# Ascend-Research/HeadPoseEstimation-WHENet

Hardware: NVIDIA H100
Metric: head-crops/sec @224x224 bf16 (higher is better)
Workload: dtype bf16

## Files before the change

### headposeestimation-whenet_b200/build.py

```python
from __future__ import annotations

import os
import subprocess
import sys

HERE = os.path.dirname(os.path.abspath(__file__))
CSRC = os.path.join(HERE, "csrc")
OBJ = os.path.join(CSRC, "obj")
LIB = os.path.join(HERE, "libwhenet_b200.so")
_SIMT_TC = ["kernels_simt.cuh", "kernels_tc.cuh"]
_ABI = os.path.join("..", "..", "include", "whenet_b200.h")
UNITS = {
    "whenet_api.cu": _SIMT_TC + ["api_error.h", "kernels_fused.cuh", "kernels_crop.cuh", "kernels_k2.cuh", "kernels_tc32.cuh", "kernels_dwse.cuh", _ABI],
    "inst_k1_bf16.cu": _SIMT_TC + ["kernels_fused.cuh"],
    "inst_k1_f16.cu": _SIMT_TC + ["kernels_fused.cuh"],
    "inst_dwse.cu": _SIMT_TC + ["kernels_fused.cuh", "kernels_dwse.cuh"],
    "inst_pw.cu": _SIMT_TC + ["kernels_fused.cuh", "kernels_k2.cuh"],
    "inst_yolo.cu": _SIMT_TC + ["kernels_yolo.cuh"],
    "yolo_api.cu": _SIMT_TC + ["kernels_yolo.cuh", "api_error.h", _ABI],
}
SOURCES = list(UNITS)
HEADERS = sorted({h for hs in UNITS.values() for h in hs})

NVCC_FLAGS = ["-O3", "-std=c++17", "-gencode", "arch=compute_90a,code=sm_90a", "-lineinfo", "-Xcompiler", "-fPIC"]


def _obj(src: str) -> str:
    return os.path.join(OBJ, os.path.splitext(src)[0] + ".o")


def _unit_stale(src: str) -> bool:
    o = _obj(src)
    if not os.path.exists(o):
        return True
    t = os.path.getmtime(o)
    deps = [os.path.join(CSRC, d) for d in [src] + UNITS[src]] + [os.path.abspath(__file__)]
    return any(os.path.exists(d) and os.path.getmtime(d) > t for d in deps)


def _stale() -> bool:
    if not os.path.exists(LIB):
        return True
    t = os.path.getmtime(LIB)
    deps = [os.path.join(CSRC, d) for d in SOURCES + HEADERS] + [os.path.abspath(__file__)]
    return any(os.path.exists(d) and os.path.getmtime(d) > t for d in deps)


# ... 31 lines not shown
```

### headposeestimation-whenet_b200/csrc/inst_k1_bf16.cu

```cuda
#include "kernels_fused.cuh"

namespace whenet {
namespace fused {
template int launch_k1<__nv_bfloat16>(cudaStream_t, K1Params, int, int, int, int, size_t, int);
template int launch_dw_only<__nv_bfloat16>(cudaStream_t, K1Params, size_t, int);
}
}
```

### headposeestimation-whenet_b200/csrc/kernels_fused.cuh

```cuda
#pragma once
#include <algorithm>

#include "kernels_tc.cuh"

namespace whenet {
namespace fused {

using tc::BK;
using tc::BM;

constexpr size_t K1_MAX_SMEM = 227 * 1024 - 256;
constexpr float kDwScale = 4.0f;

struct K1Params {
    const void* in;
    const void* wt_aug;
    const float* w_dw;
    const void* w_dw16;
    const float* b_dw;
    void* out;
    float* partial;
    const float *w_se1t, *b_se1, *w_se2, *b_se2;
    float* gate;
    int* se_counter;
// ... 38 lines not shown
}
__device__ __forceinline__ void ffma2(float2& d, const float2& a, const float2& b) {
    d.x = fmaf(a.x, b.x, d.x);
    d.y = fmaf(a.y, b.y, d.y);
}
template <typename T> __device__ __forceinline__ void unpack2(uint32_t u, float& lo, float& hi);
template <> __device__ __forceinline__ void unpack2<__nv_bfloat16>(uint32_t u, float& lo, float& hi) {
    lo = __uint_as_float(u << 16);
    hi = __uint_as_float(u & 0xffff0000u);
}
template <> __device__ __forceinline__ void unpack2<__half>(uint32_t u, float& lo, float& hi) {
    const float2 f = __half22float2(*reinterpret_cast<const __half2*>(&u));
    lo = f.x; hi = f.y;
}
template <typename T> __device__ __forceinline__ uint32_t pack2(float lo, float hi);
template <> __device__ __forceinline__ uint32_t pack2<__nv_bfloat16>(float lo, float hi) {
    const __nv_bfloat162 h = __floats2bfloat162_rn(lo, hi);
    return *reinterpret_cast<const uint32_t*>(&h);
}
template <> __device__ __forceinline__ uint32_t pack2<__half>(float lo, float hi) {
    const __half2 h = __floats2half2_rn(lo, hi);
    return *reinterpret_cast<const uint32_t*>(&h);
}
template <typename T> __device__ __forceinline__ uint32_t ones2();
template <> __device__ __forceinline__ uint32_t ones2<__nv_bfloat16>() { return 0x3f803f80u; }
template <> __device__ __forceinline__ uint32_t ones2<__half>() { return 0x3c003c00u; }

__device__ __forceinline__ uint32_t sw128(int r, int c) {
    return (uint32_t)((r >> 3) * 1024 + (r & 7) * 128 + ((c ^ (r & 7)) << 4));
}

__device__ __forceinline__ int div_small(int x, float inv) { return __float2int_rz(((float)x + 0.5f) * inv); }

template <typename T, int KS, int S, int R, bool NOEXP = false, int CCT = 0, int NT = 256>
__global__ void __launch_bounds__(NT, NT == 256 ? 2 : 1) k1_expand_dw_kernel(const K1Params p) {
    const int CC = CCT ? CCT : p.CC;
    const int pitchE = CCT ? CCT * 2 + 16 : p.pitchE;
    constexpr bool HDW = !NOEXP && std::is_same<T, __nv_bfloat16>::value;
    constexpr int NG = NT / 128;
    extern __shared__ uint8_t smem_raw[];
    __shared__ int s_last;

    const int tid = threadIdx.x, warp = tid >> 5, lane = tid & 31;
    const uint32_t smem0 = (tc::smem_u32(smem_raw) + 1023u) & ~1023u;
    const uint32_t sA = smem0;
    const uint32_t sW = sA + p.smem_A;
    const uint32_t sC = sW + 2 * p.smem_W;
    const uint32_t sE = sC + 2 * p.smem_C;
    const uint32_t sR = sE + p.smem_E;
    float* const sM = reinterpret_cast<float*>(smem_raw + (sR + (uint32_t)(p.PY * CC) * 4u - tc::smem_u32(smem_raw)));

    const T* in = reinterpret_cast<const T*>(p.in);
    const T* wt = reinterpret_cast<const T*>(p.wt_aug);
    T* out = reinterpret_cast<T*>(p.out);

    const int n0 = blockIdx.y * p.NB, tile = blockIdx.x;
    const int nb_here = min(p.NB, p.N - n0);
    const int tyi = div_small(tile, 1.0f / (float)p.tiles_x);
    const int ty0 = tyi * p.TH, tx0 = (tile - tyi * p.tiles_x) * p.TW;
    const int iy0 = ty0 * S - p.pad, ix0 = tx0 * S - p.pad;
    const int npix = p.IH * p.IW;
    const int ty_lo = max(0, -iy0), tx_lo = max(0, -ix0);
    const int IHin = min(p.IH, p.Hin - iy0) - ty_lo, IWin = min(p.IW, p.Hin - ix0) - tx_lo;
    const int npix_in = IHin * IWin;
    const int rows_gemm = nb_here * npix_in;
    const float inv_IWin = 1.0f / (float)IWin, inv_npix = 1.0f / (float)npix_in;
// ... 92 lines not shown
    const int nstrips = p.TH << p.spr_log2;
    const uint32_t e_rowstride = (uint32_t)p.IW * pitchE;
    constexpr int NCOL = (R - 1) * S + KS;
    T* const out_n = out + (long long)(n0 + jc) * p.Ho * p.Ho * p.Cexp;

    asm volatile("cp.async.wait_group 0;" ::: "memory");
    asm volatile("fence.proxy.async.shared::cta;" ::: "memory");
    __syncthreads();
    constexpr bool BF16 = std::is_same<T, __nv_bfloat16>::value;
    const int nch16 = CC >> 4;
    constexpr int kMaxPieces = CCT ? CCT / 16 : 8;

    for (int ch = ch_begin; ch < ch_end; ++ch) {
        const int buf = ch & 1;
        const int cbase = ch * CC;
        if (!NOEXP) {
            for (int u = grp; u * 64 < rows_gemm; u += NG) {
                float d[8 * kMaxPieces];
                if constexpr (CCT != 0) {
                    tc::wg_mma_m64<BF16, CCT>(d, sA + (uint32_t)u * 64 * 128, a_kb_stride, sW + buf * p.smem_W, (uint32_t)CC * 128, p.cpr >> 1);
                } else {
#pragma unroll
                    for (int jj = 0; jj < kMaxPieces; ++jj)
                        if (jj < nch16)
                            tc::wg_mma_m64<BF16, 16>(*reinterpret_cast<float(*)[8]>(d + 8 * jj), sA + (uint32_t)u * 64 * 128, a_kb_stride,
                                                     sW + buf * p.smem_W + (uint32_t)jj * 2048u, (uint32_t)CC * 128, p.cpr >> 1);
                }
                tc::wg_wait<0>();
                const int r_lo = u * 64 + 16 * wq + (lane >> 2), cq = 2 * (lane & 3);
#pragma unroll
                for (int hr = 0; hr < 2; ++hr) {
                    const int r = r_lo + 8 * hr;
                    if (r < rows_gemm) {
                        const uint32_t er = e_row_of(r);
#pragma unroll
                        for (int jj = 0; jj < kMaxPieces; ++jj) {
                            if (jj < nch16) {
#pragma unroll
                                for (int i = 0; i < 2; ++i) {
                                    const uint32_t v = pack2<__half>(swish_from_half(d[8 * jj + 4 * i + 2 * hr]), swish_from_half(d[8 * jj + 4 * i + 2 * hr + 1]));
                                    asm volatile("st.shared.b32 [%0], %1;" ::"r"(er + (uint32_t)(16 * jj + 8 * i + cq) * 2u), "r"(v) : "memory");
                                }
                            }
                        }
                    }
                }
            }
        }
        if (ch + 1 < ch_end) prefetch_c(ch + 1, buf ^ 1);
        asm volatile("cp.async.commit_group;" ::: "memory");
        asm volatile("cp.async.wait_group 0;" ::: "memory");
        asm volatile("fence.proxy.async.shared::cta;" ::: "memory");
        __syncthreads();
        if (ch + 2 < ch_end) prefetch_w(ch + 2, buf);
        asm volatile("cp.async.commit_group;" ::: "memory");

        float sum[4] = {0.f, 0.f, 0.f, 0.f};
        if (dw_active) {
            const int c0 = cbase + cv * 4;
            const uint32_t cst = sC + buf * p.smem_C + (uint32_t)cv * 16;
            const float4 bq = lds_f4(cst);
            const uint32_t e_cv = sE + (uint32_t)(jc * p.e_rows) * pitchE + (uint32_t)cv * 8;
            for (int sidx = pl; sidx < nstrips; sidx += p.PYc) {
                const int oyl = sidx >> p.spr_log2, oxl0 = (sidx - (oyl << p.spr_log2)) * R;
                float2 acc[R][2];
                uint32_t erow = e_cv + (uint32_t)(oyl * S) * e_rowstride + (uint32_t)(oxl0 * S) * pitchE;
                using TE = typename std::conditional<NOEXP, T, __half>::type;
                if constexpr (!HDW) {
#pragma unroll
                    for (int r = 0; r < R; ++r) { acc[r][0] = make_float2(bq.x, bq.y); acc[r][1] = make_float2(bq.z, bq.w); }
#pragma unroll
                    for (int ky = 0; ky < KS; ++ky) {
                        float2 wr[KS][2];
#pragma unroll
                        for (int kx = 0; kx < KS; ++kx) {
                            const float4 wq = lds_f4(cst + (uint32_t)((1 + ky * KS + kx) * CC) * 4);
                            wr[kx][0] = make_float2(wq.x, wq.y); wr[kx][1] = make_float2(wq.z, wq.w);
                        }
                        uint32_t ea = erow;
#pragma unroll
                        for (int col = 0; col < NCOL; ++col) {
                            uint32_t a, b;
                            lds64(ea, a, b);
                            ea += pitchE;
                            float2 x01, x23;
                            unpack2<TE>(a, x01.x, x01.y);
                            unpack2<TE>(b, x23.x, x23.y);
#pragma unroll
                            for (int r = 0; r < R; ++r) {
                                const int kx = col - r * S;
                                if (kx >= 0 && kx < KS) {
                                    ffma2(acc[r][0], x01, wr[kx][0]);
                                    ffma2(acc[r][1], x23, wr[kx][1]);
                                }
                            }
                        }
                        erow += e_rowstride;
                    }
                } else {
                    __half2 hacc[R][2];
#pragma unroll
                    for (int r = 0; r < R; ++r) { hacc[r][0] = __float2half2_rn(0.f); hacc[r][1] = __float2half2_rn(0.f); }
                    const uint32_t cst_h = cst - (uint32_t)cv * 16 + (uint32_t)CC * 4 + (uint32_t)cv * 8;
#pragma unroll
                    for (int ky = 0; ky < KS; ++ky) {
                        __half2 wr[KS][2];
#pragma unroll
                        for (int kx = 0; kx < KS; ++kx) {
                            uint32_t w0, w1;
                            lds64(cst_h + (uint32_t)((ky * KS + kx) * CC) * 2, w0, w1);
                            wr[kx][0] = *reinterpret_cast<__half2*>(&w0); wr[kx][1] = *reinterpret_cast<__half2*>(&w1);
                        }
                        uint32_t ea = erow;
#pragma unroll
                        for (int col = 0; col < NCOL; ++col) {
                            uint32_t a, b;
                            lds64(ea, a, b);
                            ea += pitchE;
                            const __half2 x01 = *reinterpret_cast<__half2*>(&a), x23 = *reinterpret_cast<__half2*>(&b);
#pragma unroll
                            for (int r = 0; r < R; ++r) {
                                const int kx = col - r * S;
                                if (kx >= 0 && kx < KS) {
                                    hacc[r][0] = __hfma2(x01, wr[kx][0], hacc[r][0]);
                                    hacc[r][1] = __hfma2(x23, wr[kx][1], hacc[r][1]);
                                }
                            }
                        }
                        erow += e_rowstride;
                    }
                    const float2 sc = make_float2(kDwScale, kDwScale);
#pragma unroll
                    for (int r = 0; r < R; ++r) {
                        acc[r][0] = make_float2(bq.x, bq.y); acc[r][1] = make_float2(bq.z, bq.w);
                        ffma2(acc[r][0], __half22float2(hacc[r][0]), sc);
                        ffma2(acc[r][1], __half22float2(hacc[r][1]), sc);
                    }
                }
                const int oy = ty0 + oyl;
                T* dst = out_n + ((long long)oy * p.Ho + tx0 + oxl0) * p.Cexp + c0;
#pragma unroll
                for (int r = 0; r < R; ++r) {
                    if (oxl0 + r < p.TW && oy < p.Ho && tx0 + oxl0 + r < p.Ho) {
#pragma unroll
                        for (int i = 0; i < 2; ++i) {
                            acc[r][i].x = swish_from_half(acc[r][i].x); acc[r][i].y = swish_from_half(acc[r][i].y);
                            sum[2 * i] += acc[r][i].x; sum[2 * i + 1] += acc[r][i].y;
                        }
                        uint2 o;
                        o.x = pack2<T>(acc[r][0].x, acc[r][0].y);
                        o.y = pack2<T>(acc[r][1].x, acc[r][1].y);
                        *reinterpret_cast<uint2*>(dst + (long long)r * p.Cexp) = o;
                    }
                }
            }
            asm volatile("st.shared.v4.f32 [%0], {%1,%2,%3,%4};" ::"r"(sR + (uint32_t)(py * CC + cv * 4) * 4),
                         "f"(sum[0]), "f"(sum[1]), "f"(sum[2]), "f"(sum[3]) : "memory");
        }
        __syncthreads();
        if (tid < p.NB * CC) {
            const int jj = tid >= CC ? 1 : 0, cc = tid - jj * CC;
            if (jj < nb_here) {
                float s4[4] = {0.f, 0.f, 0.f, 0.f};
                const uint32_t r0 = sR + (uint32_t)(jj * p.PYc * CC + cc) * 4;
                int y = 0;
                for (; y + 3 < p.PYc; y += 4) {
#pragma unroll
                    for (int i = 0; i < 4; ++i) {
                        float t;
                        asm volatile("ld.shared.f32 %0, [%1];" : "=f"(t) : "r"(r0 + (uint32_t)((y + i) * CC) * 4));
                        s4[i] += t;
                    }
                }
                for (; y < p.PYc; ++y) {
                    float t;
                    asm volatile("ld.shared.f32 %0, [%1];" : "=f"(t) : "r"(r0 + (uint32_t)(y * CC) * 4));
                    s4[y & 3] += t;
                }
                const float tot = (s4[0] + s4[1]) + (s4[2] + s4[3]);
                p.partial[((long long)(n0 + jj) * gridDim.x + tile) * p.Cexp + cbase + cc] = tot;
                if (p.se_tail) sM[jj * p.Cexp + cbase + cc] = tot * p.inv_hw;
            }
        }
        __syncthreads();
    }
    if (p.se_counter) __threadfence();
    __syncthreads();
// ... 202 lines not shown
```

### headposeestimation-whenet_b200/csrc/whenet_api.cu

```cuda
#include <cuda_bf16.h>
#include <cuda_fp16.h>
#include <cuda_runtime.h>

#include <algorithm>
#include <atomic>
#include <cmath>
#include <cstdarg>
#include <cstdio>
#include <cstdlib>
#include <cstring>
#include <map>
#include <string>
#include <thread>
#include <type_traits>
#include <vector>

#include "../../include/whenet_b200.h"
#include "api_error.h"
#include "kernels_simt.cuh"
#include "kernels_tc.cuh"
#include "kernels_fused.cuh"
#include "kernels_crop.cuh"
#include "kernels_k2.cuh"
#include "kernels_tc32.cuh"
#include "kernels_dwse.cuh"
#include <cudaTypedefs.h>

namespace whenet {
namespace fused {
#define WHENET_EXTERN_FUSED(T)                                                                            \
    extern template int launch_k1<T>(cudaStream_t, K1Params, int, int, int, int, size_t, int);            \
    extern template int launch_dw_only<T>(cudaStream_t, K1Params, size_t, int);
WHENET_EXTERN_FUSED(__nv_bfloat16)
WHENET_EXTERN_FUSED(__half)
#undef WHENET_EXTERN_FUSED
extern template int launch_dwse<__nv_bfloat16>(cudaStream_t, DwSeParams, int, int, int, int, int);
extern template int launch_dwse_x<__nv_bfloat16>(cudaStream_t, DwSeParams, int, int, int, int, int);
extern template int launch_dwse_spatial<__nv_bfloat16>(cudaStream_t, DwSeParams, int, int, int);
}
namespace tc {
#define WHENET_EXTERN_PW(T)                                                                                                         \
    extern template int launch_pw_tc2<T>(cudaStream_t, const T*, const void*, const float*, const float*, const T*, T*, long long, \
                                         int, int, int, bool, int, int, int, bool);                                                 \
    extern template int launch_k2<T>(cudaStream_t, const K2Params&, size_t, bool, bool, bool, int);          \
    extern template int launch_pw_tc3<T>(cudaStream_t, const T*, const void*, const float*, const float*, const T*, T*, long long, int, int, int);
WHENET_EXTERN_PW(__nv_bfloat16)
WHENET_EXTERN_PW(__half)
#undef WHENET_EXTERN_PW
}
}

namespace {

using whenet::api::fail;
using whenet::api::g_err;

#define CK(call)                                                                                   \
    do {                                                                                           \
        cudaError_t e__ = (call);                                                                  \
        if (e__ != cudaSuccess)                                                                    \
            return fail(WHENET_ECUDA, "%s failed at %s:%d: %s", #call, __FILE__, __LINE__,         \
                        cudaGetErrorString(e__));                                                  \
    } while (0)

constexpr double kBnEps = 1e-3;
constexpr int kImgElems = 224 * 224 * 3;

struct BlockCfg {
    int idx, hin, hout, cin, cexp, cout, k, s, cse, pad;
    bool skip, has_expand;
};
// ... 51 lines not shown
struct GraphEntry { GraphKey key; cudaGraphExec_t exec; int launches; };
struct EvPair { cudaEvent_t a, b; int stat; };
struct Stat { std::string name; double bytes = 0, flops = 0; int launches = 0; float ms = 0; };

}

struct whenet_ctx {
    int device = 0, max_batch = 0, precision = 0;
    int chunk = 0;
    int use_tc = 0;
    int* h_tflag = nullptr;
    int* d_tflag = nullptr;
    int dw_variant = 1;
    int pw_variant = 4;
    std::map<TmapKey, CUtensorMap> tmaps2;
    int pw_stage_cap = 0, pw_smem_kb = 54, pw_min_ctas = 132;
    int stem_variant = 1;
    whenet::StemParams stem_params{};
    bool async_host = false;
    unsigned host_pass_ctr = 0;
    float* d_angles_slot[2] = {nullptr, nullptr};
    float* d_logits_slot[2] = {nullptr, nullptr};
    int host_chunk = 1 << 30;
    int cfg_epoch = 0;
    int use_graph = 0;
    std::vector<GraphEntry> graphs;
    int use_fused = 0;
    int fused_max_block = 16;
    int kd_tail = 0;
    int se_batch = 1;
    int pw3 = 1;
    int dw1_kd = 1;
    int head_batch = 1;
    int kd_from = 7;
    std::vector<K1Plan> k1;
    std::map<TmapKey, CUtensorMap> tmaps;
    int sm_count = 132;
    K1Plan dw1;
    int dw1_fused = 1;
    cudaStream_t own_stream = nullptr, stream = nullptr, copy_stream = nullptr;
    bool weights_loaded = false;
    std::vector<BlockCfg> blocks;
    std::vector<BlockW> bw;
    float* d_arena = nullptr;
    void* d_arena16 = nullptr;
    size_t split_lo_bytes = 0;
    std::vector<int64_t> layout;
    float *w_stem = nullptr, *b_stem = nullptr, *lut = nullptr;
    float *w_head = nullptr, *b_head = nullptr, *w_fct = nullptr, *b_fc = nullptr;
    void* wt_head = nullptr;
    int ws_chunk = 0;
    size_t ws_io = 0, ws_ex = 0, ws_dw = 0, ws_part = 0;
    cudaStream_t aux_stream[4] = {nullptr, nullptr, nullptr, nullptr};
    cudaEvent_t ev_fork = nullptr, ev_join[4] = {nullptr, nullptr, nullptr, nullptr}, ev_half[4] = {nullptr, nullptr, nullptr, nullptr};
    int n_streams = 2;
    void *bufA = nullptr, *bufB = nullptr, *bufE = nullptr, *bufD = nullptr;
    float *d_partial = nullptr, *d_gate = nullptr, *d_angles = nullptr, *d_logits = nullptr, *d_pooled = nullptr;
    int* d_se_counter = nullptr;
    int se_wide = 0;
    int se_scale_out = 1;
    int k1_split_ctas = 120;
    int se_tail = 1;
    int se_fused = 0;
    void* d_in[2] = {nullptr, nullptr};
    void* h_stage = nullptr;
    size_t h_stage_bytes = 0;
// ... 141 lines not shown
    static PFN_cuTensorMapEncodeTiled_v12000 fn = nullptr;
    if (!fn) {
        void* f = nullptr;
        cudaDriverEntryPointQueryResult q;
        if (cudaGetDriverEntryPoint("cuTensorMapEncodeTiled", &f, cudaEnableDefault, &q) == cudaSuccess && q == cudaDriverEntryPointSuccess)
            fn = reinterpret_cast<PFN_cuTensorMapEncodeTiled_v12000>(f);
    }
    return fn;
}
int make_tmap_w(CUtensorMap* tm, const void* base, int rows, int K, int box_rows, bool is_bf16) {
    auto fn = tmap_encode_fn();
    if (!fn) return fail(WHENET_ECUDA, "cuTensorMapEncodeTiled is not available from this driver");
    const cuuint64_t dims[2] = {(cuuint64_t)K, (cuuint64_t)rows};
    const cuuint64_t strides[1] = {(cuuint64_t)K * 2};
    const cuuint32_t box[2] = {64, (cuuint32_t)box_rows};
    const cuuint32_t estr[2] = {1, 1};
    const CUresult r = fn(tm, is_bf16 ? CU_TENSOR_MAP_DATA_TYPE_BFLOAT16 : CU_TENSOR_MAP_DATA_TYPE_FLOAT16, 2, const_cast<void*>(base), dims, strides,
                          box, estr, CU_TENSOR_MAP_INTERLEAVE_NONE, CU_TENSOR_MAP_SWIZZLE_128B, CU_TENSOR_MAP_L2_PROMOTION_L2_256B,
                          CU_TENSOR_MAP_FLOAT_OOB_FILL_NONE);
    if (r != CUDA_SUCCESS) return fail(WHENET_ECUDA, "cuTensorMapEncodeTiled(weights %dx%d, box %d) failed: %d", rows, K, box_rows, (int)r);
    return 0;
}

int make_tmap_kd_e(CUtensorMap* tm, const void* base, int n, int H, int C, int cc, int pw) {
    auto fn = tmap_encode_fn();
    if (!fn) return fail(WHENET_ECUDA, "cuTensorMapEncodeTiled is not available from this driver");
    const cuuint64_t dims[4] = {(cuuint64_t)C, (cuuint64_t)H, (cuuint64_t)H, (cuuint64_t)n};
    const cuuint64_t strides[3] = {(cuuint64_t)C * 2, (cuuint64_t)H * C * 2, (cuuint64_t)H * H * C * 2};
    const cuuint32_t box[4] = {(cuuint32_t)cc, (cuuint32_t)pw, (cuuint32_t)pw, 1};
    const cuuint32_t estr[4] = {1, 1, 1, 1};
    const CUresult r = fn(tm, CU_TENSOR_MAP_DATA_TYPE_FLOAT16, 4, const_cast<void*>(base), dims, strides, box, estr, CU_TENSOR_MAP_INTERLEAVE_NONE,
                          CU_TENSOR_MAP_SWIZZLE_NONE, CU_TENSOR_MAP_L2_PROMOTION_L2_128B, CU_TENSOR_MAP_FLOAT_OOB_FILL_NONE);
    if (r != CUDA_SUCCESS) return fail(WHENET_ECUDA, "cuTensorMapEncodeTiled(KD tile %dx%dx%dx%d, box %dx%dx%d) failed: %d", n, H, H, C, pw, pw, cc, (int)r);
    return 0;
}
int make_tmap_kd_w(CUtensorMap* tm, const void* base, int kk, int C, int cc) {
    auto fn = tmap_encode_fn();
    if (!fn) return fail(WHENET_ECUDA, "cuTensorMapEncodeTiled is not available from this driver");
    const cuuint64_t dims[2] = {(cuuint64_t)C, (cuuint64_t)kk};
    const cuuint64_t strides[1] = {(cuuint64_t)C * 2};
    const cuuint32_t box[2] = {(cuuint32_t)cc, (cuuint32_t)kk};
    const cuuint32_t estr[2] = {1, 1};
    const CUresult r = fn(tm, CU_TENSOR_MAP_DATA_TYPE_FLOAT16, 2, const_cast<void*>(base), dims, strides, box, estr, CU_TENSOR_MAP_INTERLEAVE_NONE,
                          CU_TENSOR_MAP_SWIZZLE_NONE, CU_TENSOR_MAP_L2_PROMOTION_L2_128B, CU_TENSOR_MAP_FLOAT_OOB_FILL_NONE);
    if (r != CUDA_SUCCESS) return fail(WHENET_ECUDA, "cuTensorMapEncodeTiled(KD weights %dx%d, box %d) failed: %d", kk, C, cc, (int)r);
    return 0;
}

template <typename T>
int launch_pw(whenet_ctx* c, const char* name, const T* A, const float* W, const void* Wt16, const float* bias,
              const float* gate, const T* resid, T* out, long long M, int K, int N, int hw, bool swish, bool out_half = false) {
    const double bytes = (double)M * (K + N + (resid ? N : 0)) * sizeof(T);
    const double flops = 2.0 * (double)M * K * N;
    Scope sc(c, name, bytes, flops);
    if constexpr (sizeof(T) == 2) {
        const bool want_k2 = c->pw_variant == 3 || (c->pw_variant == 4 && (gate == nullptr || hw <= 196));
        if (c->use_tc && Wt16 && want_k2 && !out_half) {
            whenet::tc::K2Params kp{};
            size_t smem = 0;
            if (whenet::tc::plan_k2(M, K, N, hw, gate != nullptr, c->precision == WHENET_PRECISION_BF16, &kp, &smem) &&
                (c->pw_variant == 3 || kp.tiles >= 2 * c->sm_count)) {
                if (c->tmaps2.size() > 1024) c->tmaps2.clear();
                const TmapKey ka{K, (int)M, (const void*)A}, kw{-N, K, Wt16};
                auto ia = c->tmaps2.find(ka);
                if (ia == c->tmaps2.end()) {
                    CUtensorMap tm;
// ... 235 lines not shown
                    if (rc != 0) return fail(WHENET_ECUDA, "KD (on-chip expand) launch failed for block %d (rc=%d)", b.idx, rc);
                    CK(cudaGetLastError());
                } else {
                    Scope sc(c, nm, (double)nb * ((double)b.hin * b.hin + (double)b.hout * b.hout) * b.cexp * sizeof(T),
                             2.0 * nb * (double)b.hout * b.hout * b.k * b.k * b.cexp);
                    rc = whenet::fused::launch_dwse<T>(c->stream, p, b.k, b.s, b.hin, nb, split);
                    if (rc != 0) return fail(WHENET_ECUDA, "KD launch failed for block %d (rc=%d)", b.idx, rc);
                    CK(cudaGetLastError());
                }
                tiles = 1;
                did_k1 = true;
              }
            } else if (c->use_fused && c->k1[i].valid && b.idx <= c->fused_max_block) {
                whenet::fused::K1Params p = c->k1[i].p;
                p.in = cur; p.wt_aug = w.wt_exp_aug; p.w_dw = w.w_dw_h; p.w_dw16 = w.w_dw16; p.b_dw = w.b_dw_h; p.out = D; p.partial = c->d_partial; p.tflag = c->d_tflag;
                p.w_se1t = w.w_se1t; p.b_se1 = w.b_se1; p.w_se2 = w.w_se2; p.b_se2 = w.b_se2; p.gate = c->d_gate; p.Cse = b.cse;
                se_in_k1 = c->se_fused && p.NB == 1;
                p.se_counter = se_in_k1 ? c->d_se_counter : nullptr;
                {
                    const long long ctas = (long long)p.tiles_x * p.tiles_y * ((nb + p.NB - 1) / p.NB);
                    int split = 1;
                    while (split < p.n_chunks && ctas * split < c->k1_split_ctas) ++split;
                    p.chunks_per_cta = (p.n_chunks + split - 1) / split;
                    if (c->se_tail && !se_in_k1 && p.tiles_x * p.tiles_y == 1 && split == 1) {
                        p.se_tail = 1;
                        p.inv_hw = 1.0f / (float)(b.hout * b.hout);
                        se_in_k1 = true;
                        if (c->se_scale_out && !taps) { p.scale_out = 1; d_gated = true; }
                    }
                }
                snprintf(nm, sizeof nm, "b%02d.k1", b.idx);
                Scope sc(c, nm, (double)nb * ((double)b.hin * b.hin * b.cin + (double)b.hout * b.hout * b.cexp) * sizeof(T),
                         2.0 * nb * ((double)b.hin * b.hin * b.cin * b.cexp + (double)b.hout * b.hout * b.k * b.k * b.cexp));
                int rc = whenet::fused::launch_k1<T>(c->stream, p, b.k, b.s, c->k1[i].R, c->k1[i].NT, c->k1[i].smem, nb);
                if (rc != 0) return fail(WHENET_ECUDA, "K1 launch failed for block %d (rc=%d)", b.idx, rc);
                CK(cudaGetLastError());
                tiles = p.tiles_x * p.tiles_y;
                did_k1 = true;
            }
        }
        if (!did_k1) {
        if (b.has_expand) {
            snprintf(nm, sizeof nm, "b%02d.expand", b.idx);
            int rc = launch_pw<T>(c, nm, cur, w.w_exp, w.wt_exp, w.b_exp, nullptr, nullptr, E,
                                  (long long)nb * b.hin * b.hin, b.cin, b.cexp, b.hin * b.hin, true);
            if (rc) return rc;
            dw_in = E;
        }
        snprintf(nm, sizeof nm, "b%02d.dw", b.idx);
        int rc = launch_dw<T>(c, nm, b, w, dw_in, D, nb, &tiles);
        if (rc) return rc;
        }
        int rc = 0;
        if (!se_in_k1) {
            snprintf(nm, sizeof nm, "b%02d.se", b.idx);
            Scope sc(c, nm, (double)nb * (tiles + 1) * b.cexp * 4.0, 4.0 * nb * b.cexp * b.cse);
            const float inv_hw = 1.0f / (float)(b.hout * b.hout);
            const size_t se_smem = (b.cexp + b.cse) * sizeof(float);
            if (nb >= 64 && c->se_batch) {
                constexpr int SEB = 4;
                whenet::se_gate_batch_kernel<SEB, 512><<<(nb + SEB - 1) / SEB, 512, SEB * se_smem, c->stream>>>(
                    c->d_partial, tiles, inv_hw, w.w_se1t, w.b_se1, w.w_se2, w.b_se2, c->d_gate, b.cexp, b.cse, nb);
            } else if (nb < 64 || c->se_wide)
                whenet::se_gate_kernel<1024><<<nb, 1024, se_smem, c->stream>>>(
                    c->d_partial, tiles, inv_hw, w.w_se1t, w.b_se1, w.w_se2, w.b_se2, c->d_gate, b.cexp, b.cse);
            else
                whenet::se_gate_kernel<256><<<nb, 256, se_smem, c->stream>>>(
                    c->d_partial, tiles, inv_hw, w.w_se1t, w.b_se1, w.w_se2, w.b_se2, c->d_gate, b.cexp, b.cse);
            CK(cudaGetLastError());
// ... 404 lines not shown
    if (prop.major != 9 || prop.minor != 0)
        return fail(WHENET_ECUDA, "device %d is sm_%d%d; this library is built for sm_90a (H100) only", device, prop.major, prop.minor);
    whenet_ctx* c = new whenet_ctx();
    c->device = device;
    c->max_batch = max_batch;
    c->precision = precision;
    c->sm_count = prop.multiProcessorCount;
    const char* ev = getenv("WHENET_CHUNK");
    int chunk = ev ? atoi(ev) : max_batch;
    if (chunk < 1) chunk = max_batch;
    c->chunk = std::min(chunk, max_batch);
    c->use_tc = precision != WHENET_PRECISION_FP32;
    if (const char* e2 = getenv("WHENET_TC")) c->use_tc = atoi(e2) && precision != WHENET_PRECISION_FP32;
    c->blocks = make_blocks();
    c->bw.resize(c->blocks.size());
    c->k1.resize(c->blocks.size());
    if (precision != WHENET_PRECISION_FP32) {
        const BlockCfg& b1 = c->blocks[0];
        c->dw1.valid = !b1.has_expand && whenet::fused::plan_dw_only(b1.hin, b1.cexp, b1.k, b1.s, b1.pad, &c->dw1.p, &c->dw1.smem);
        c->dw1.R = 7;
    }
    if (precision != WHENET_PRECISION_FP32)
        for (size_t i = 0; i < c->blocks.size(); ++i) {
            const BlockCfg& b = c->blocks[i];
            if (!b.has_expand) continue;
            K1Plan& pl = c->k1[i];
            whenet::fused::K1Choice ch{};
            pl.valid = whenet::fused::plan_k1(b.hin, b.hout, b.cin, b.cexp, b.k, b.s, b.pad, precision == WHENET_PRECISION_BF16, true,
                                              &pl.p, &ch, &pl.smem);
            pl.R = ch.r;
            pl.NT = ch.nt;
        }
    c->use_fused = precision != WHENET_PRECISION_FP32;
    if (const char* e3 = getenv("WHENET_FUSED")) c->use_fused = atoi(e3) && precision != WHENET_PRECISION_FP32;
    CK(cudaStreamCreateWithFlags(&c->own_stream, cudaStreamNonBlocking));
    CK(cudaStreamCreateWithFlags(&c->copy_stream, cudaStreamNonBlocking));
    c->stream = c->own_stream;
    CK(cudaEventCreateWithFlags(&c->ev_fork, cudaEventDisableTiming));
    for (int i = 0; i < 4; ++i) {
        CK(cudaStreamCreateWithFlags(&c->aux_stream[i], cudaStreamNonBlocking));
        CK(cudaEventCreateWithFlags(&c->ev_join[i], cudaEventDisableTiming));
        CK(cudaEventCreateWithFlags(&c->ev_half[i], cudaEventDisableTiming));
    }
    for (int i = 0; i < 2; ++i) {
        CK(cudaEventCreateWithFlags(&c->ev_ready[i], cudaEventDisableTiming));
        CK(cudaEventCreateWithFlags(&c->ev_free[i], cudaEventDisableTiming));
    }
    CK(cudaHostAlloc((void**)&c->h_tflag, sizeof(int), cudaHostAllocMapped));
    *c->h_tflag = 0;
    CK(cudaHostGetDevicePointer((void**)&c->d_tflag, c->h_tflag, 0));
    CK(cudaMalloc(&c->d_angles, (size_t)max_batch * 3 * sizeof(float) * 2));
    CK(cudaMalloc(&c->d_logits, (size_t)max_batch * WHENET_N_LOGITS * sizeof(float) * 2));
    for (int i = 0; i < 2; ++i) {
        c->d_angles_slot[i] = c->d_angles + (size_t)i * max_batch * 3;
        c->d_logits_slot[i] = c->d_logits + (size_t)i * max_batch * WHENET_N_LOGITS;
    }
    *out = c;
    return 0;
}

int whenet_load_weights(whenet_ctx* c, const whenet_tensor* tensors, int n_tensors) {
    if (!c || !tensors || n_tensors < 1) return fail(WHENET_EINVAL, "bad arguments");
    CK(cudaSetDevice(c->device));
    TensorMap tm;
    for (int i = 0; i < n_tensors; ++i)
        if (tensors[i].name) tm.m[tensors[i].name] = &tensors[i];
// ... 433 lines not shown
            out[n].ms = s.ms; out[n].launches = s.launches; out[n].bytes = s.bytes; out[n].flops = s.flops;
        }
        ++n;
    }
    if (out) { c->stats.clear(); c->stat_idx.clear(); }
    return n;
}

int64_t whenet_launch_count(whenet_ctx* c) { return c ? c->launches : 0; }

int whenet_set_option(whenet_ctx* c, const char* key, int value) {
    if (!c || !key) return fail(WHENET_EINVAL, "bad arguments");
    drop_graphs(c);
    c->cfg_epoch++;
    if (!strcmp(key, "tensor_cores")) { c->use_tc = value; return 0; }
    if (!strcmp(key, "streams")) { c->n_streams = value < 1 ? 1 : (value > 4 ? 4 : value); return 0; }
    if (!strcmp(key, "se_fused")) { c->se_fused = value; return 0; }
    if (!strcmp(key, "se_tail")) { c->se_tail = value; return 0; }
    if (!strcmp(key, "se_scale_out")) { c->se_scale_out = value; return 0; }
    if (!strcmp(key, "k1_split_ctas")) { c->k1_split_ctas = value; return 0; }
    if (!strcmp(key, "se_wide")) { c->se_wide = value; return 0; }
    if (!strcmp(key, "host_chunk")) { if (value < 1) return fail(WHENET_EINVAL, "host_chunk must be >= 1"); c->host_chunk = value; return 0; }
    if (!strcmp(key, "graph")) { c->use_graph = value; if (!value) drop_graphs(c); return 0; }
    if (!strcmp(key, "dw_variant")) { c->dw_variant = value; return 0; }
    if (!strcmp(key, "stem_variant")) { c->stem_variant = value; return 0; }
    if (!strcmp(key, "dw1_fused")) { c->dw1_fused = value; return 0; }
    if (!strcmp(key, "pw_variant")) { c->pw_variant = value; return 0; }
    if (!strcmp(key, "pw_stage_cap")) { c->pw_stage_cap = value; return 0; }
    if (!strcmp(key, "pw_smem_kb")) { c->pw_smem_kb = value; return 0; }
    if (!strcmp(key, "pw_min_ctas")) { c->pw_min_ctas = value; return 0; }
    if (!strcmp(key, "fused")) { c->use_fused = value && c->precision != WHENET_PRECISION_FP32; return 0; }
    if (!strcmp(key, "fused_max_block")) { c->fused_max_block = value; return 0; }
    if (!strcmp(key, "kd_from")) { c->kd_from = value; return 0; }
    if (!strcmp(key, "kd_tail")) { c->kd_tail = value; return 0; }
    if (!strcmp(key, "se_batch")) { c->se_batch = value; return 0; }
    if (!strcmp(key, "head_batch")) { c->head_batch = value; return 0; }
    if (!strcmp(key, "dw1_kd")) { c->dw1_kd = value; return 0; }
    if (!strcmp(key, "pw3")) { c->pw3 = value; return 0; }
    if (!strcmp(key, "stage_threads")) { c->stage_threads = value < 0 ? 0 : (value > 32 ? 32 : value); return 0; }
    if (!strcmp(key, "chunk")) {
        if (value < 1) return fail(WHENET_EINVAL, "chunk must be >= 1");
        c->chunk = std::min(value, c->max_batch);
        return 0;
    }
    return fail(WHENET_ENOTFOUND, "unknown option %s", key);
}

void whenet_destroy(whenet_ctx* c) {
    if (!c) return;
    cudaSetDevice(c->device);
    cudaDeviceSynchronize();
    drop_graphs(c);
    free_ws(c);
    if (c->d_frame) cudaFree(c->d_frame);
    if (c->d_rects) cudaFree(c->d_rects);
    if (c->d_frame_of) cudaFree(c->d_frame_of);
    for (auto& kv : c->taps) cudaFree(kv.second.first);
    for (auto& p : c->ev_used) { cudaEventDestroy(p.a); cudaEventDestroy(p.b); }
    for (auto e : c->ev_pool) cudaEventDestroy(e);
    if (c->d_arena) cudaFree(c->d_arena);
    if (c->d_arena16) cudaFree(c->d_arena16);
    if (c->d_angles) cudaFree(c->d_angles);
    if (c->d_logits) cudaFree(c->d_logits);
    if (c->h_tflag) cudaFreeHost(c->h_tflag);
    for (int i = 0; i < 2; ++i) {
        if (c->ev_ready[i]) cudaEventDestroy(c->ev_ready[i]);
// ... 17 lines not shown
```

Before: 74410.

## Add specialized TMA-fed expand+depthwise K1X kernel for bf16 blocks

Adds a new compile-time specialized kernel that fuses the expand GEMM (wgmma) and HFMA2 depthwise conv for selected block shapes. All operands are loaded by TMA with mbarrier pipelining: the input tile, double-buffered expand weights and double-buffered depthwise weights plus bias. It also factors the shared expand-store and depthwise strip code into helpers reused by the old kernel. The intent is to cut per-thread address math and manual staging loads and to overlap weight fetch with compute. The cost is more template instances, extra tensor-map management, and a path taken only when a shape instance matches.

```diff
diff --git a/headposeestimation-whenet_b200/build.py b/headposeestimation-whenet_b200/build.py
--- a/headposeestimation-whenet_b200/build.py
+++ b/headposeestimation-whenet_b200/build.py
@@ -11,8 +11,8 @@
 _SIMT_TC = ["kernels_simt.cuh", "kernels_tc.cuh"]
 _ABI = os.path.join("..", "..", "include", "whenet_b200.h")
 UNITS = {
-    "whenet_api.cu": _SIMT_TC + ["api_error.h", "kernels_fused.cuh", "kernels_crop.cuh", "kernels_k2.cuh", "kernels_tc32.cuh", "kernels_dwse.cuh", _ABI],
-    "inst_k1_bf16.cu": _SIMT_TC + ["kernels_fused.cuh"],
+    "whenet_api.cu": _SIMT_TC + ["api_error.h", "kernels_fused.cuh", "kernels_crop.cuh", "kernels_k2.cuh", "kernels_tc32.cuh", "kernels_dwse.cuh", "kernels_k1x.cuh", _ABI],
+    "inst_k1_bf16.cu": _SIMT_TC + ["kernels_fused.cuh", "kernels_dwse.cuh", "kernels_k1x.cuh"],
     "inst_k1_f16.cu": _SIMT_TC + ["kernels_fused.cuh"],
     "inst_dwse.cu": _SIMT_TC + ["kernels_fused.cuh", "kernels_dwse.cuh"],
     "inst_pw.cu": _SIMT_TC + ["kernels_fused.cuh", "kernels_k2.cuh"],
diff --git a/headposeestimation-whenet_b200/csrc/inst_k1_bf16.cu b/headposeestimation-whenet_b200/csrc/inst_k1_bf16.cu
--- a/headposeestimation-whenet_b200/csrc/inst_k1_bf16.cu
+++ b/headposeestimation-whenet_b200/csrc/inst_k1_bf16.cu
@@ -1,8 +1,10 @@
 #include "kernels_fused.cuh"
+#include "kernels_k1x.cuh"
 
 namespace whenet {
 namespace fused {
 template int launch_k1<__nv_bfloat16>(cudaStream_t, K1Params, int, int, int, int, size_t, int);
 template int launch_dw_only<__nv_bfloat16>(cudaStream_t, K1Params, size_t, int);
+template int launch_k1x<__nv_bfloat16>(cudaStream_t, DwSeParams, int, int, int, int, int, int, int, int);
 }
 }
diff --git a/headposeestimation-whenet_b200/csrc/kernels_fused.cuh b/headposeestimation-whenet_b200/csrc/kernels_fused.cuh
--- a/headposeestimation-whenet_b200/csrc/kernels_fused.cuh
+++ b/headposeestimation-whenet_b200/csrc/kernels_fused.cuh
@@ -94,6 +94,81 @@
 
 __device__ __forceinline__ int div_small(int x, float inv) { return __float2int_rz(((float)x + 0.5f) * inv); }
 
+template <int NP>
+__device__ __forceinline__ void expand_row_to_e(const float (&d)[8 * NP], int nch16, int hr, uint32_t er, int cq) {
+#pragma unroll
+    for (int jj = 0; jj < NP; ++jj) {
+        if (jj < nch16) {
+#pragma unroll
+            for (int i = 0; i < 2; ++i) {
+                const uint32_t v = pack2<__half>(swish_from_half(d[8 * jj + 4 * i + 2 * hr]), swish_from_half(d[8 * jj + 4 * i + 2 * hr + 1]));
+                asm volatile("st.shared.b32 [%0], %1;" ::"r"(er + (uint32_t)(16 * jj + 8 * i + cq) * 2u), "r"(v) : "memory");
+            }
+        }
+    }
+}
+
+template <int KS, int S, int R>
+__device__ __forceinline__ void dw_strip_hfma2(uint32_t erow, uint32_t e_rowstride, uint32_t pitchE, uint32_t wts, uint32_t w_pitch,
+                                               const float4& bq, float2 (&acc)[R][2]) {
+    constexpr int NCOL = (R - 1) * S + KS;
+    __half2 hacc[R][2];
+#pragma unroll
+    for (int r = 0; r < R; ++r) { hacc[r][0] = __float2half2_rn(0.f); hacc[r][1] = __float2half2_rn(0.f); }
+#pragma unroll
+    for (int ky = 0; ky < KS; ++ky) {
+        __half2 wr[KS][2];
+#pragma unroll
+        for (int kx = 0; kx < KS; ++kx) {
+            uint32_t w0, w1;
+            lds64(wts + (uint32_t)(ky * KS + kx) * w_pitch, w0, w1);
+            wr[kx][0] = *reinterpret_cast<__half2*>(&w0); wr[kx][1] = *reinterpret_cast<__half2*>(&w1);
+        }
+        uint32_t ea = erow;
+#pragma unroll
+        for (int col = 0; col < NCOL; ++col) {
+            uint32_t a, b;
+            lds64(ea, a, b);
+            ea += pitchE;
+            const __half2 x01 = *reinterpret_cast<__half2*>(&a), x23 = *reinterpret_cast<__half2*>(&b);
+#pragma unroll
+            for (int r = 0; r < R; ++r) {
+                const int kx = col - r * S;
+                if (kx >= 0 && kx < KS) {
+                    hacc[r][0] = __hfma2(x01, wr[kx][0], hacc[r][0]);
+                    hacc[r][1] = __hfma2(x23, wr[kx][1], hacc[r][1]);
+                }
+            }
+        }
+        erow += e_rowstride;
+    }
+    const float2 sc = make_float2(kDwScale, kDwScale);
+#pragma unroll
+    for (int r = 0; r < R; ++r) {
+        acc[r][0] = make_float2(bq.x, bq.y); acc[r][1] = make_float2(bq.z, bq.w);
+        ffma2(acc[r][0], __half22float2(hacc[r][0]), sc);
+        ffma2(acc[r][1], __half22float2(hacc[r][1]), sc);
+    }
+}
+
+template <typename T, int R>
+__device__ __forceinline__ void dw_strip_finish(float2 (&acc)[R][2], int nvalid, T* dst, int Cexp, float (&sum)[4]) {
+#pragma unroll
+    for (int r = 0; r < R; ++r) {
+        if (r < nvalid) {
+#pragma unroll
+            for (int i = 0; i < 2; ++i) {
+                acc[r][i].x = swish_from_half(acc[r][i].x); acc[r][i].y = swish_from_half(acc[r][i].y);
+                sum[2 * i] += acc[r][i].x; sum[2 * i + 1] += acc[r][i].y;
+            }
+            uint2 o;
+            o.x = pack2<T>(acc[r][0].x, acc[r][0].y);
+            o.y = pack2<T>(acc[r][1].x, acc[r][1].y);
+            *reinterpret_cast<uint2*>(dst + (long long)r * Cexp) = o;
+        }
+    }
+}
+
 template <typename T, int KS, int S, int R, bool NOEXP = false, int CCT = 0, int NT = 256>
 __global__ void __launch_bounds__(NT, NT == 256 ? 2 : 1) k1_expand_dw_kernel(const K1Params p) {
     const int CC = CCT ? CCT : p.CC;
@@ -252,17 +327,7 @@
                 for (int hr = 0; hr < 2; ++hr) {
                     const int r = r_lo + 8 * hr;
                     if (r < rows_gemm) {
-                        const uint32_t er = e_row_of(r);
-#pragma unroll
-                        for (int jj = 0; jj < kMaxPieces; ++jj) {
-                            if (jj < nch16) {
-#pragma unroll
-                                for (int i = 0; i < 2; ++i) {
-                                    const uint32_t v = pack2<__half>(swish_from_half(d[8 * jj + 4 * i + 2 * hr]), swish_from_half(d[8 * jj + 4 * i + 2 * hr + 1]));
-                                    asm volatile("st.shared.b32 [%0], %1;" ::"r"(er + (uint32_t)(16 * jj + 8 * i + cq) * 2u), "r"(v) : "memory");
-                                }
-                            }
-                        }
+                        expand_row_to_e<kMaxPieces>(d, nch16, hr, e_row_of(r), cq);
                     }
                 }
             }
@@ -318,61 +383,12 @@
                         erow += e_rowstride;
                     }
                 } else {
-                    __half2 hacc[R][2];
-#pragma unroll
-                    for (int r = 0; r < R; ++r) { hacc[r][0] = __float2half2_rn(0.f); hacc[r][1] = __float2half2_rn(0.f); }
-                    const uint32_t cst_h = cst - (uint32_t)cv * 16 + (uint32_t)CC * 4 + (uint32_t)cv * 8;
-#pragma unroll
-                    for (int ky = 0; ky < KS; ++ky) {
-                        __half2 wr[KS][2];
-#pragma unroll
-                        for (int kx = 0; kx < KS; ++kx) {
-                            uint32_t w0, w1;
-                            lds64(cst_h + (uint32_t)((ky * KS + kx) * CC) * 2, w0, w1);
-                            wr[kx][0] = *reinterpret_cast<__half2*>(&w0); wr[kx][1] = *reinterpret_cast<__half2*>(&w1);
-                        }
-                        uint32_t ea = erow;
-#pragma unroll
-                        for (int col = 0; col < NCOL; ++col) {
-                            uint32_t a, b;
-                            lds64(ea, a, b);
-                            ea += pitchE;
-                            const __half2 x01 = *reinterpret_cast<__half2*>(&a), x23 = *reinterpret_cast<__half2*>(&b);
-#pragma unroll
-                            for (int r = 0; r < R; ++r) {
-                                const int kx = col - r * S;
-                                if (kx >= 0 && kx < KS) {
-                                    hacc[r][0] = __hfma2(x01, wr[kx][0], hacc[r][0]);
-                                    hacc[r][1] = __hfma2(x23, wr[kx][1], hacc[r][1]);
-                                }
-                            }
-                        }
-                        erow += e_rowstride;
-                    }
-                    const float2 sc = make_float2(kDwScale, kDwScale);
-#pragma unroll
-                    for (int r = 0; r < R; ++r) {
-                        acc[r][0] = make_float2(bq.x, bq.y); acc[r][1] = make_float2(bq.z, bq.w);
-                        ffma2(acc[r][0], __half22float2(hacc[r][0]), sc);
-                        ffma2(acc[r][1], __half22float2(hacc[r][1]), sc);
-                    }
+                    dw_strip_hfma2<KS, S, R>(erow, e_rowstride, (uint32_t)pitchE, cst - (uint32_t)cv * 16 + (uint32_t)CC * 4 + (uint32_t)cv * 8,
+                                             (uint32_t)CC * 2, bq, acc);
                 }
                 const int oy = ty0 + oyl;
                 T* dst = out_n + ((long long)oy * p.Ho + tx0 + oxl0) * p.Cexp + c0;
-#pragma unroll
-                for (int r = 0; r < R; ++r) {
-                    if (oxl0 + r < p.TW && oy < p.Ho && tx0 + oxl0 + r < p.Ho) {
-#pragma unroll
-                        for (int i = 0; i < 2; ++i) {
-                            acc[r][i].x = swish_from_half(acc[r][i].x); acc[r][i].y = swish_from_half(acc[r][i].y);
-                            sum[2 * i] += acc[r][i].x; sum[2 * i + 1] += acc[r][i].y;
-                        }
-                        uint2 o;
-                        o.x = pack2<T>(acc[r][0].x, acc[r][0].y);
-                        o.y = pack2<T>(acc[r][1].x, acc[r][1].y);
-                        *reinterpret_cast<uint2*>(dst + (long long)r * p.Cexp) = o;
-                    }
-                }
+                dw_strip_finish<T, R>(acc, oy < p.Ho ? min(p.TW - oxl0, p.Ho - tx0 - oxl0) : 0, dst, p.Cexp, sum);
             }
             asm volatile("st.shared.v4.f32 [%0], {%1,%2,%3,%4};" ::"r"(sR + (uint32_t)(py * CC + cv * 4) * 4),
                          "f"(sum[0]), "f"(sum[1]), "f"(sum[2]), "f"(sum[3]) : "memory");
diff --git a/headposeestimation-whenet_b200/csrc/kernels_k1x.cuh b/headposeestimation-whenet_b200/csrc/kernels_k1x.cuh
--- /dev/null
+++ b/headposeestimation-whenet_b200/csrc/kernels_k1x.cuh
@@ -0,0 +1,175 @@
+#pragma once
+#include "kernels_dwse.cuh"
+
+namespace whenet {
+namespace fused {
+
+template <int KS, int S, int HIN, int TH, int R, int CC, int CIN>
+struct K1X {
+    static constexpr int NT = 256;
+    static constexpr int HO = (HIN + S - 1) / S;
+    static constexpr int PAD = ((HO - 1) * S + KS - HIN > 0 ? (HO - 1) * S + KS - HIN : 0) / 2;
+    static constexpr int TILES_X = HO / TH, TILES = TILES_X * TILES_X;
+    static constexpr int IW = (TH - 1) * S + KS;
+    static constexpr int NPIX = IW * IW;
+    static constexpr int HALVES = (NPIX + 63) / 64;
+    static constexpr int KCH = CIN / 8;
+    static constexpr int KSTEPS = ((KCH + 2) & ~1) >> 1;
+    static constexpr int SPR = (TH + R - 1) / R;
+    static constexpr int NSTRIPS = TH * SPR;
+    static constexpr int CV = CC / 4;
+    static constexpr int PY = NT / CV;
+    static constexpr uint32_t PITCHE = CC * 2 + 16;
+    static constexpr int E_ROWS = NPIX + R * S + 16;
+    static_assert(HO % TH == 0 && CIN % 8 == 0 && KCH + 1 < 8 && CC % 16 == 0 && CC <= 128, "tile plan");
+    static constexpr uint32_t A_BYTES = (NPIX + 7) / 8 * 8 * 128;
+    static constexpr uint32_t A_TX = NPIX * 128;
+    static constexpr uint32_t W_BYTES = CC * 128;
+    static constexpr uint32_t E_BYTES = (E_ROWS * PITCHE + 127) / 128 * 128;
+    static constexpr uint32_t DWW_BYTES = KS * KS * CC * 2;
+    static constexpr uint32_t CST_TX = DWW_BYTES + CC * 4;
+    static constexpr uint32_t CST_BYTES = (CST_TX + 127) / 128 * 128;
+    static constexpr uint32_t RED_BYTES = PY * CC * 4;
+    static constexpr uint32_t OFF_W = A_BYTES, OFF_E = OFF_W + 2 * W_BYTES, OFF_C = OFF_E + E_BYTES, OFF_R = OFF_C + 2 * CST_BYTES;
+    static constexpr size_t SMEM = (size_t)OFF_R + 2 * RED_BYTES + 1024;
+    static_assert((A_BYTES | W_BYTES) % 1024 == 0 && DWW_BYTES % 16 == 0, "operand alignment");
+    static_assert((size_t)HALVES * 64 * 128 + 1024 <= SMEM, "the last half's MMA stays inside the CTA's window");
+    static_assert(2 * (SMEM + 1024 + 64) <= 228 * 1024, "two CTAs per SM");
+};
+
+template <int KS, int S, int HIN, int TH, int R, int CC, int CIN>
+__global__ void __launch_bounds__(256, 2) k1x_kernel(const __grid_constant__ DwSeParams p) {
+    using X = K1X<KS, S, HIN, TH, R, CC, CIN>;
+    using T = __nv_bfloat16;
+    extern __shared__ uint8_t smem_k1x[];
+    __shared__ __align__(8) uint64_t bars[5];
+    __shared__ int s_abort_mem;
+    volatile int* s_abort = &s_abort_mem;
+    const uint32_t s0 = (tc::smem_u32(smem_k1x) + 1023u) & ~1023u;
+    const uint32_t sA = s0, sW = s0 + X::OFF_W, sE = s0 + X::OFF_E, sC = s0 + X::OFF_C, sR = s0 + X::OFF_R;
+    const uint32_t b_a = tc::smem_u32(&bars[0]), b_w = b_a + 8, b_c = b_a + 24;
+
+    const int tid = threadIdx.x, warp = tid >> 5, lane = tid & 31;
+    const int wg = tid >> 7, wq = warp & 3;
+    const int tile = blockIdx.x, n = blockIdx.y;
+    const int tyi = tile / X::TILES_X;
+    const int ty0 = tyi * TH, tx0 = (tile - tyi * X::TILES_X) * TH;
+    const int iy0 = ty0 * S - X::PAD, ix0 = tx0 * S - X::PAD;
+    const int C = p.C, n_chunks = p.n_chunks;
+
+    if (tid == 0) {
+        for (int i = 0; i < 5; ++i) tc::mbar_init(&bars[i], 1);
+        s_abort_mem = 0;
+        asm volatile("fence.mbarrier_init.release.cluster;" ::: "memory");
+        asm volatile("prefetch.tensormap [%0];" ::"l"(&p.tmX) : "memory");
+        asm volatile("prefetch.tensormap [%0];" ::"l"(&p.tmWx) : "memory");
+        asm volatile("prefetch.tensormap [%0];" ::"l"(&p.tmW) : "memory");
+    }
+    __syncthreads();
+
+    auto issue_w = [&](int j) {
+        const uint32_t bar = b_w + 8 * (j & 1);
+        tc::mbar::arrive_expect_tx(bar, X::W_BYTES);
+        tc::mbar::tma_2d(sW + (j & 1) * X::W_BYTES, &p.tmWx, 0, j * CC, bar);
+    };
+    auto issue_c = [&](int j) {
+        const uint32_t bar = b_c + 8 * (j & 1), dst = sC + (j & 1) * X::CST_BYTES;
+        tc::mbar::arrive_expect_tx(bar, X::CST_TX);
+        tc::mbar::tma_2d(dst, &p.tmW, j * CC, 0, bar);
+        asm volatile("cp.async.bulk.shared::cluster.global.mbarrier::complete_tx::bytes [%0], [%1], %2, [%3];"
+                     ::"r"(dst + X::DWW_BYTES), "l"(p.b_dw + j * CC), "r"((uint32_t)(CC * 4)), "r"(bar) : "memory");
+    };
+    if (tid == 0) {
+        tc::mbar::arrive_expect_tx(b_a, X::A_TX);
+        tc::mbar::tma_4d(sA, &p.tmX, 0, ix0, iy0, n, b_a);
+        issue_w(0); issue_c(0);
+        if (n_chunks > 1) { issue_w(1); issue_c(1); }
+    }
+
+    const int py = tid / X::CV, cv = tid - py * X::CV;
+    const bool dw_active = py < X::PY;
+    T* const out_t = reinterpret_cast<T*>(p.out) + (((long long)n * X::HO + ty0) * X::HO + tx0) * C + cv * 4;
+
+    tc::mbar::wait(b_a, 0, s_abort, p.tflag);
+    for (int r = tid; r < X::NPIX; r += X::NT) {
+        const int ty = r / X::IW, tx = r - ty * X::IW;
+        const int iy = iy0 + ty, ix = ix0 + tx;
+        if (iy >= 0 && iy < HIN && ix >= 0 && ix < HIN) sts128(sA + sw128(r, X::KCH), make_uint4(ones2<T>(), 0u, 0u, 0u));
+    }
+    asm volatile("fence.proxy.async.shared::cta;" ::: "memory");
+    __syncthreads();
+
+    for (int j = 0; j < n_chunks; ++j) {
+        const int buf = j & 1;
+        const uint32_t par = (uint32_t)(j >> 1) & 1u;
+        tc::mbar::wait(b_w + 8 * buf, par, s_abort, p.tflag);
+        for (int u = wg; u < X::HALVES; u += 2) {
+            float d[CC / 2];
+            tc::wg_mma_m64<true, CC>(d, sA + (uint32_t)u * 64 * 128, X::A_BYTES, sW + buf * X::W_BYTES, X::W_BYTES, X::KSTEPS);
+            tc::wg_wait<0>();
+            const int r_lo = u * 64 + 16 * wq + (lane >> 2), cq = 2 * (lane & 3);
+#pragma unroll
+            for (int hr = 0; hr < 2; ++hr) {
+                const int r = r_lo + 8 * hr;
+                if (r < X::NPIX) expand_row_to_e<CC / 16>(d, CC / 16, hr, sE + (uint32_t)r * X::PITCHE, cq);
+            }
+        }
+        __syncthreads();
+        if (tid == 0 && j + 2 < n_chunks) issue_w(j + 2);
+
+        tc::mbar::wait(b_c + 8 * buf, par, s_abort, p.tflag);
+        if (dw_active && !*s_abort) {
+            const uint32_t cst = sC + buf * X::CST_BYTES;
+            const float4 bq = lds_f4(cst + X::DWW_BYTES + (uint32_t)cv * 16);
+            float sum[4] = {0.f, 0.f, 0.f, 0.f};
+            for (int sidx = py; sidx < X::NSTRIPS; sidx += X::PY) {
+                const int oyl = sidx / X::SPR, oxl0 = (sidx - oyl * X::SPR) * R;
+                float2 acc[R][2];
+                dw_strip_hfma2<KS, S, R>(sE + (uint32_t)((oyl * S * X::IW + oxl0 * S) * X::PITCHE + cv * 8), X::IW * X::PITCHE, X::PITCHE,
+                                         cst + (uint32_t)cv * 8, CC * 2, bq, acc);
+                dw_strip_finish<T, R>(acc, TH - oxl0, out_t + ((long long)oyl * X::HO + oxl0) * C + j * CC, C, sum);
+            }
+            asm volatile("st.shared.v4.f32 [%0], {%1,%2,%3,%4};" ::"r"(sR + (uint32_t)(buf * X::RED_BYTES + (py * CC + cv * 4) * 4)),
+                         "f"(sum[0]), "f"(sum[1]), "f"(sum[2]), "f"(sum[3]) : "memory");
+        }
+        __syncthreads();
+        if (warp == X::NT / 32 - 1) {
+            squeeze_sums<X::PY, CC>(sR + buf * X::RED_BYTES, p.partial + ((long long)n * X::TILES + tile) * C + j * CC, nullptr, 0.f, lane);
+            if (lane == 0 && j + 2 < n_chunks) issue_c(j + 2);
+        }
+    }
+}
+
+#define WHENET_K1X_INSTANCES(F) F(3, 2, 112, 8, 4, 48, 16) F(3, 1, 56, 14, 7, 48, 24) F(5, 2, 56, 7, 4, 48, 24) F(3, 2, 28, 7, 7, 80, 40)
+
+inline bool k1x_has_instance(int k, int s, int hin, int cin, int pad, const K1Params& pl, int R) {
+#define K1X_MATCH(KS_, S_, HIN_, TH_, R_, CC_, CIN_)                                                                        \
+    if (k == KS_ && s == S_ && hin == HIN_ && cin == CIN_ && pl.TH == TH_ && pl.TW == TH_ && R == R_ && pl.CC == CC_ && pl.NB == 1 && \
+        pad == K1X<KS_, S_, HIN_, TH_, R_, CC_, CIN_>::PAD)                                                                  \
+        return true;
+    WHENET_K1X_INSTANCES(K1X_MATCH)
+#undef K1X_MATCH
+    return false;
+}
+
+template <typename T>
+int launch_k1x(cudaStream_t stream, DwSeParams p, int k, int s, int hin, int cin, int th, int r, int cc, int n_crops) {
+    static_assert(std::is_same<T, __nv_bfloat16>::value, "K1X runs the bf16 wgmma and the HFMA2 depthwise");
+    p.N = n_crops;
+    p.n_chunks = p.C / cc;
+    p.chunks_per_cta = p.n_chunks;
+#define K1X_GO(KS, S, HIN, TH, RR, CC, CIN)                                                                                  \
+    if (k == KS && s == S && hin == HIN && cin == CIN && th == TH && r == RR && cc == CC) {                                  \
+        using X = K1X<KS, S, HIN, TH, RR, CC, CIN>;                                                                          \
+        auto kfn = k1x_kernel<KS, S, HIN, TH, RR, CC, CIN>;                                                                  \
+        if (cudaFuncSetAttribute(kfn, cudaFuncAttributeMaxDynamicSharedMemorySize, (int)X::SMEM) != cudaSuccess) return -1;  \
+        kfn<<<dim3(X::TILES, n_crops), X::NT, X::SMEM, stream>>>(p);                                                         \
+        return 0;                                                                                                            \
+    }
+    WHENET_K1X_INSTANCES(K1X_GO)
+#undef K1X_GO
+    return 1;
+}
+
+}
+}
diff --git a/headposeestimation-whenet_b200/csrc/whenet_api.cu b/headposeestimation-whenet_b200/csrc/whenet_api.cu
--- a/headposeestimation-whenet_b200/csrc/whenet_api.cu
+++ b/headposeestimation-whenet_b200/csrc/whenet_api.cu
@@ -24,6 +24,7 @@
 #include "kernels_k2.cuh"
 #include "kernels_tc32.cuh"
 #include "kernels_dwse.cuh"
+#include "kernels_k1x.cuh"
 #include <cudaTypedefs.h>
 
 namespace whenet {
@@ -37,6 +38,7 @@
 extern template int launch_dwse<__nv_bfloat16>(cudaStream_t, DwSeParams, int, int, int, int, int);
 extern template int launch_dwse_x<__nv_bfloat16>(cudaStream_t, DwSeParams, int, int, int, int, int);
 extern template int launch_dwse_spatial<__nv_bfloat16>(cudaStream_t, DwSeParams, int, int, int);
+extern template int launch_k1x<__nv_bfloat16>(cudaStream_t, DwSeParams, int, int, int, int, int, int, int, int);
 }
 namespace tc {
 #define WHENET_EXTERN_PW(T)                                                                                                         \
@@ -154,6 +156,7 @@
     int pw3 = 1;
     int dw1_kd = 1;
     int head_batch = 1;
+    int k1x = 0;
     int kd_from = 7;
     std::vector<K1Plan> k1;
     std::map<TmapKey, CUtensorMap> tmaps;
@@ -361,6 +364,18 @@
     const CUresult r = fn(tm, CU_TENSOR_MAP_DATA_TYPE_FLOAT16, 4, const_cast<void*>(base), dims, strides, box, estr, CU_TENSOR_MAP_INTERLEAVE_NONE,
                           CU_TENSOR_MAP_SWIZZLE_NONE, CU_TENSOR_MAP_L2_PROMOTION_L2_128B, CU_TENSOR_MAP_FLOAT_OOB_FILL_NONE);
     if (r != CUDA_SUCCESS) return fail(WHENET_ECUDA, "cuTensorMapEncodeTiled(KD tile %dx%dx%dx%d, box %dx%dx%d) failed: %d", n, H, H, C, pw, pw, cc, (int)r);
+    return 0;
+}
+int make_tmap_k1x_in(CUtensorMap* tm, const void* base, int n, int H, int C, int iw) {
+    auto fn = tmap_encode_fn();
+    if (!fn) return fail(WHENET_ECUDA, "cuTensorMapEncodeTiled is not available from this driver");
+    const cuuint64_t dims[4] = {(cuuint64_t)C, (cuuint64_t)H, (cuuint64_t)H, (cuuint64_t)n};
+    const cuuint64_t strides[3] = {(cuuint64_t)C * 2, (cuuint64_t)H * C * 2, (cuuint64_t)H * H * C * 2};
+    const cuuint32_t box[4] = {64, (cuuint32_t)iw, (cuuint32_t)iw, 1};
+    const cuuint32_t estr[4] = {1, 1, 1, 1};
+    const CUresult r = fn(tm, CU_TENSOR_MAP_DATA_TYPE_BFLOAT16, 4, const_cast<void*>(base), dims, strides, box, estr, CU_TENSOR_MAP_INTERLEAVE_NONE,
+                          CU_TENSOR_MAP_SWIZZLE_128B, CU_TENSOR_MAP_L2_PROMOTION_L2_128B, CU_TENSOR_MAP_FLOAT_OOB_FILL_NONE);
+    if (r != CUDA_SUCCESS) return fail(WHENET_ECUDA, "cuTensorMapEncodeTiled(K1X input %dx%dx%dx%d, box %dx%d) failed: %d", n, H, H, C, iw, iw, (int)r);
     return 0;
 }
 int make_tmap_kd_w(CUtensorMap* tm, const void* base, int kk, int C, int cc) {
@@ -662,9 +677,45 @@
                 snprintf(nm, sizeof nm, "b%02d.k1", b.idx);
                 Scope sc(c, nm, (double)nb * ((double)b.hin * b.hin * b.cin + (double)b.hout * b.hout * b.cexp) * sizeof(T),
                          2.0 * nb * ((double)b.hin * b.hin * b.cin * b.cexp + (double)b.hout * b.hout * b.k * b.k * b.cexp));
-                int rc = whenet::fused::launch_k1<T>(c->stream, p, b.k, b.s, c->k1[i].R, c->k1[i].NT, c->k1[i].smem, nb);
-                if (rc != 0) return fail(WHENET_ECUDA, "K1 launch failed for block %d (rc=%d)", b.idx, rc);
-                CK(cudaGetLastError());
+                bool did_k1x = false;
+                if constexpr (std::is_same<T, __nv_bfloat16>::value) {
+                    if (c->k1x && c->use_tc && p.chunks_per_cta == p.n_chunks && !se_in_k1 &&
+                        whenet::fused::k1x_has_instance(b.k, b.s, b.hin, b.cin, b.pad, p, c->k1[i].R)) {
+                        whenet::fused::DwSeParams q{};
+                        int rc = 0;
+                        if (c->tmaps.size() > 512) c->tmaps.clear();
+                        const TmapKey kx{600 + b.idx, nb, (const void*)cur}, kwx{700 + b.idx, 0, (const void*)w.wt_exp_aug}, kw{500 + b.idx, 0, (const void*)w.w_dw16};
+                        auto ix = c->tmaps.find(kx);
+                        if (ix == c->tmaps.end()) {
+                            CUtensorMap tm;
+                            if ((rc = make_tmap_k1x_in(&tm, cur, nb, b.hin, b.cin, p.IW))) return rc;
+                            ix = c->tmaps.emplace(kx, tm).first;
+                        }
+                        auto iwx = c->tmaps.find(kwx);
+                        if (iwx == c->tmaps.end()) {
+                            CUtensorMap tm;
+                            if ((rc = make_tmap_w(&tm, w.wt_exp_aug, b.cexp, b.cin + 8, p.CC, true))) return rc;
+                            iwx = c->tmaps.emplace(kwx, tm).first;
+                        }
+                        auto iw = c->tmaps.find(kw);
+                        if (iw == c->tmaps.end()) {
+                            CUtensorMap tm;
+                            if ((rc = make_tmap_kd_w(&tm, w.w_dw16, b.k * b.k, b.cexp, p.CC))) return rc;
+                            iw = c->tmaps.emplace(kw, tm).first;
+                        }
+                        q.tmX = ix->second; q.tmWx = iwx->second; q.tmW = iw->second;
+                        q.b_dw = w.b_dw_h; q.tflag = c->d_tflag; q.out = D; q.partial = c->d_partial; q.C = b.cexp; q.pad = b.pad;
+                        rc = whenet::fused::launch_k1x<T>(c->stream, q, b.k, b.s, b.hin, b.cin, p.TH, c->k1[i].R, p.CC, nb);
+                        if (rc != 0) return fail(WHENET_ECUDA, "K1X launch failed for block %d (rc=%d)", b.idx, rc);
+                        CK(cudaGetLastError());
+                        did_k1x = true;
+                    }
+                }
+                if (!did_k1x) {
+                    int rc = whenet::fused::launch_k1<T>(c->stream, p, b.k, b.s, c->k1[i].R, c->k1[i].NT, c->k1[i].smem, nb);
+                    if (rc != 0) return fail(WHENET_ECUDA, "K1 launch failed for block %d (rc=%d)", b.idx, rc);
+                    CK(cudaGetLastError());
+                }
                 tiles = p.tiles_x * p.tiles_y;
                 did_k1 = true;
             }
@@ -1135,6 +1186,7 @@
             pl.NT = ch.nt;
         }
     c->use_fused = precision != WHENET_PRECISION_FP32;
+    c->k1x = precision == WHENET_PRECISION_BF16;
     if (const char* e3 = getenv("WHENET_FUSED")) c->use_fused = atoi(e3) && precision != WHENET_PRECISION_FP32;
     CK(cudaStreamCreateWithFlags(&c->own_stream, cudaStreamNonBlocking));
     CK(cudaStreamCreateWithFlags(&c->copy_stream, cudaStreamNonBlocking));
@@ -1634,6 +1686,7 @@
     if (!strcmp(key, "fused")) { c->use_fused = value && c->precision != WHENET_PRECISION_FP32; return 0; }
     if (!strcmp(key, "fused_max_block")) { c->fused_max_block = value; return 0; }
     if (!strcmp(key, "kd_from")) { c->kd_from = value; return 0; }
+    if (!strcmp(key, "k1x")) { c->k1x = value && c->precision == WHENET_PRECISION_BF16; return 0; }
     if (!strcmp(key, "kd_tail")) { c->kd_tail = value; return 0; }
     if (!strcmp(key, "se_batch")) { c->se_batch = value; return 0; }
     if (!strcmp(key, "head_batch")) { c->head_batch = value; return 0; }
```

Result: faster. 80020, median of 6 (+7.5%).
